# SimonsRoad/gf-pl-slam

Measured on AMD Instinct MI355X. Metric: stereo frames/sec (2k ORB + 500 LBD, 10 GN iters), higher is better.
Workload: dtype f64

## Files before the change

gf-pl-slam_amd/csrc/gfpl_knn.hpp:

```cpp
#pragma once
#include "gfpl_device.hpp"
#include "gfpl_layout.hpp"
#include <type_traits>

namespace gfpl {

typedef int mfma_v4i __attribute__((ext_vector_type(4)));
typedef int mfma_v8i __attribute__((ext_vector_type(8)));
typedef float mfma_v16f __attribute__((ext_vector_type(16)));

template <int CELL>
constexpr int knn_ksteps() { return (CELL == 2 ? 512 : 256) / 64; }

typedef mfma_v16f knn_acc_t;
constexpr float KNN_ACC_BIAS = 12582912.0f;
__device__ __forceinline__ uint32_t knn_acc_bits(float a) {
    return __float_as_uint(a);
}
__device__ __forceinline__ knn_acc_t knn_mma(mfma_v4i a, mfma_v4i b, knn_acc_t c) {
    const mfma_v8i a8 = __builtin_shufflevector(a, a, 0, 1, 2, 3, -1, -1, -1, -1);
    const mfma_v8i b8 = __builtin_shufflevector(b, b, 0, 1, 2, 3, -1, -1, -1, -1);
    return __builtin_amdgcn_mfma_scale_f32_32x32x64_f8f6f4(a8, b8, c, 4, 4, 0, 0x7F7F7F7F, 0, 0x7F7F7F7F);
}

__device__ __forceinline__ uint32_t fp4_cells2(uint32_t v) {
    return (2u << (4u * (v & 3u))) | (2u << (16u + 4u * ((v >> 2) & 3u)));
}
__device__ __forceinline__ uint32_t fp4_bits8(uint32_t b) {
    uint32_t x = b & 0xFFu;
    x = (x | (x << 12)) & 0x000F000Fu;
    x = (x | (x << 6)) & 0x03030303u;
    x = (x | (x << 3)) & 0x11111111u;
    return x << 1;
}

template <int CELL, bool SIGNED>
__device__ __forceinline__ mfma_v4i knn_frag(const uint32_t* d, int ks, int h) {
    mfma_v4i f;
    if (CELL == 2) {
        const uint32_t w = d[ks] >> (8u * (uint32_t)h);
#pragma unroll
        for (int i = 0; i < 4; ++i) {
            const uint32_t x = fp4_cells2((w >> (16 * (i >> 1) + 4 * (i & 1))) & 0xFu);
            f[i] = (int)(SIGNED ? x * 5u : x);
        }
    } else {
#pragma unroll
        for (int i = 0; i < 4; ++i) {
            const uint32_t x = fp4_bits8(d[2 * ks + (i >> 1)] >> (16u * (uint32_t)h + 8u * (i & 1)));
            f[i] = (int)(SIGNED ? (x << 2) | 0x22222222u : x);
        }
    }
    return f;
}

__device__ __forceinline__ int popc8(const uint32_t* d) {
    int s = 0;
#pragma unroll
    for (int i = 0; i < 8; ++i) s += __popc(d[i]);
    return s;
}

template <int CELL>
__device__ void knn_lut_fill(uint32_t* lut) {
    for (int b = threadIdx.x; b < 256; b += blockDim.x) {
        if (CELL == 2) {
            lut[2 * b] = fp4_cells2(b & 0xFu);
            lut[2 * b + 1] = fp4_cells2((uint32_t)b >> 4);
        } else {
            lut[b] = fp4_bits8(b);
        }
    }
}

template <int CELL>
__device__ __forceinline__ void knn_stage_views(uint32_t* T, int stride, const uint8_t* src, int nt) {
    constexpr uint32_t S0 = CELL == 2 ? 0x06040200u : 0x05040100u;
    constexpr uint32_t S1 = CELL == 2 ? 0x07050301u : 0x07060302u;
    const uint4* s4 = reinterpret_cast<const uint4*>(src);
    for (int k = threadIdx.x; k < nt * 2; k += blockDim.x) {
        const uint4 v = s4[k];
        const int t = k >> 1, j = (k & 1) * 2;
        T[(0 + j) * stride + t] = __builtin_amdgcn_perm(v.y, v.x, S0);
        T[(1 + j) * stride + t] = __builtin_amdgcn_perm(v.w, v.z, S0);
        T[(4 + j) * stride + t] = __builtin_amdgcn_perm(v.y, v.x, S1);
        T[(5 + j) * stride + t] = __builtin_amdgcn_perm(v.w, v.z, S1);
    }
}


__device__ __forceinline__ knn_acc_t knn_acc_init(int off) {
    knn_acc_t c;
#pragma unroll
    for (int r = 0; r < 16; ++r) c[r] = KNN_ACC_BIAS + (float)off;
    return c;
}

template <int CELL>
__device__ __forceinline__ uint32_t knn_query_offk(const uint32_t (&qd)[8]) {
    return (uint32_t)(CELL == 2 ? 128 : popc8(qd)) << 16;
}

template <int CELL>
__device__ __forceinline__ knn_acc_t knn_tile(const uint32_t* Th, int tstride, int rt, int c, int nt, const mfma_v4i* bq,
                                              knn_acc_t acc) {
    typedef uint32_t u32x2v __attribute__((ext_vector_type(2)));
    typedef __attribute__((address_space(3))) const u32x2v lds_cu2;
    typedef __attribute__((address_space(3))) const uint32_t lds_cu1;
    const int t = rt * 32 + c;
    uint32_t tv[4];
    if (rt * 32 + 32 <= nt) {
#pragma unroll
        for (int j = 0; j < 4; ++j) tv[j] = Th[j * tstride + t];
    } else if (t < nt) {
#pragma unroll
        for (int j = 0; j < 4; ++j) tv[j] = Th[j * tstride + t];
    } else {
#pragma unroll
        for (int j = 0; j < 4; ++j) tv[j] = 0;
    }
    auto ent = [&](int i, int sh) { return (uintptr_t)(((tv[i >> 2] >> (8 * (i & 3))) & 0xFFu) << sh); };
    mfma_v4i f[knn_ksteps<CELL>()];
#pragma unroll
    for (int ks = 0; ks < knn_ksteps<CELL>(); ++ks) {
        if (CELL == 2) {
            const u32x2v e0 = *reinterpret_cast<lds_cu2*>(ent(2 * ks, 3));
            const u32x2v e1 = *reinterpret_cast<lds_cu2*>(ent(2 * ks + 1, 3));
            f[ks][0] = (int)e0.x; f[ks][1] = (int)e0.y; f[ks][2] = (int)e1.x; f[ks][3] = (int)e1.y;
        } else {
#pragma unroll
            for (int i = 0; i < 4; ++i) f[ks][i] = (int)*reinterpret_cast<lds_cu1*>(ent(4 * ks + i, 2));
        }
    }
#pragma unroll
    for (int ks = 0; ks < knn_ksteps<CELL>(); ++ks) acc = knn_mma(f[ks], bq[ks], acc);
    return acc;
}

__device__ __forceinline__ uint32_t knn_acc_row(int r) { return (uint32_t)((r & 3) + 8 * (r >> 2)); }

__device__ __forceinline__ void knn_top2(uint32_t& k0, uint32_t& k1, uint32_t key) {
    asm("v_med3_u32 %0, %1, %2, %3" : "=v"(k1) : "v"(k0), "v"(k1), "v"(key));
    k0 = min(k0, key);
}

__device__ __forceinline__ void knn_merge_halves(uint32_t& k0, uint32_t& k1) {
    const uint32_t o0 = __shfl_xor(k0, 32, 64);
    const uint32_t o1 = __shfl_xor(k1, 32, 64);
    const uint32_t lo = min(k0, o0), hi0 = max(k0, o0);
    k1 = min(hi0, min(k1, o1));
    k0 = lo;
}

template <int CELL>
__device__ __forceinline__ void knn2_mfma(const uint32_t* T, int tstride, int nt, const uint8_t* Q, int nq, uint32_t* out_k0,
                                          uint32_t* out_k1, uint32_t* rl_key) {
    const int lane = threadIdx.x & 63;
    const int wave = threadIdx.x >> 6, nwave = blockDim.x >> 6;
    const int h = lane >> 5, c = lane & 31;
    const int nct = (nq + 31) >> 5, nrt = (nt + 31) >> 5;
    typedef uint32_t u32x2v __attribute__((ext_vector_type(2)));
    typedef __attribute__((address_space(3))) const u32x2v lds_cu2;
    typedef __attribute__((address_space(3))) const uint32_t lds_cu1;
    const uint32_t* Th = T + 4 * h * tstride;
    const int pr = lane & 15;
    const bool rb3 = (pr & 8) != 0, rb2 = (pr & 4) != 0, rb1 = (pr & 2) != 0, rb0 = (pr & 1) != 0;
    const uint32_t lro = (uint32_t)(4 * h + (pr & 3) + 8 * (pr >> 2));
    knn_acc_t acc0 = knn_acc_init(0);
#pragma unroll
    for (int r = 0; r < 16; ++r) asm volatile("" : "+v"(acc0[r]));
    for (int ct = wave; ct < nct; ct += nwave) {
        const int q = ct * 32 + c;
        uint32_t qd[8];
        if (q < nq) load_desc(Q + (size_t)q * 32, qd);
        else {
#pragma unroll
            for (int i = 0; i < 8; ++i) qd[i] = 0;
        }
        mfma_v4i bq[knn_ksteps<CELL>()];
#pragma unroll
        for (int ks = 0; ks < knn_ksteps<CELL>(); ++ks) {
            bq[ks] = knn_frag<CELL, true>(qd, ks, h);
        }
        const uint32_t offk = knn_query_offk<CELL>(qd);
        const uint32_t qo = offk + (q < nq ? (uint32_t)q : 0x7FFF0000u);
        uint32_t k0 = 0xFFFFFFFFu, k1 = 0xFFFFFFFFu;
        for (int rt = 0; rt < nrt; ++rt) {
            const int t = rt * 32 + c;
            uint32_t tv[4];
            if (rt * 32 + 32 <= nt) {
#pragma unroll
                for (int j = 0; j < 4; ++j) tv[j] = Th[j * tstride + t];
            } else if (t < nt) {
#pragma unroll
                for (int j = 0; j < 4; ++j) tv[j] = Th[j * tstride + t];
            } else {
#pragma unroll
                for (int j = 0; j < 4; ++j) tv[j] = 0;
            }
            knn_acc_t acc = acc0;
#pragma unroll
            for (int ks = 0; ks < knn_ksteps<CELL>(); ++ks) {
                auto ent = [&](int i, int sh) { return (uintptr_t)(((tv[i >> 2] >> (8 * (i & 3))) & 0xFFu) << sh); };
                mfma_v4i f;
                if (CELL == 2) {
                    const u32x2v e0 = *reinterpret_cast<lds_cu2*>(ent(2 * ks, 3));
                    const u32x2v e1 = *reinterpret_cast<lds_cu2*>(ent(2 * ks + 1, 3));
                    f[0] = (int)e0.x; f[1] = (int)e0.y; f[2] = (int)e1.x; f[3] = (int)e1.y;
                } else {
#pragma unroll
                    for (int i = 0; i < 4; ++i) f[i] = (int)*reinterpret_cast<lds_cu1*>(ent(4 * ks + i, 2));
                }
                acc = knn_mma(f, bq[ks], acc);
            }
            const uint32_t tb = (uint32_t)(rt * 32 + 4 * h);
            const uint32_t tko = offk + tb;
            auto epilogue = [&](auto chk_t) {
                constexpr bool chk = decltype(chk_t)::value;
                auto top2 = [&](int r, uint32_t sh) {
                    const uint32_t ro = knn_acc_row(r);
                    uint32_t key = sh + tko + ro;
                    if (chk && (int)(tb + ro) >= nt) key = 0xFFFFFFFFu;
                    knn_top2(k0, k1, key);
                };
                auto xchg = [](uint32_t a, uint32_t b, bool upper, auto ctrl_t) {
                    const uint32_t send = upper ? a : b, keep = upper ? b : a;
                    return min(keep, (uint32_t)__builtin_amdgcn_update_dpp(-1, (int)send, decltype(ctrl_t)::value, 0xF, 0xF, false));
                };
                uint32_t y[8];
#pragma unroll
                for (int j = 0; j < 8; ++j) {
                    const uint32_t s0 = knn_acc_bits(acc[j]) << 16, s1 = knn_acc_bits(acc[j + 8]) << 16;
                    top2(j, s0);
                    top2(j + 8, s1);
                    y[j] = xchg(s0 + qo, s1 + qo, rb3, std::integral_constant<int, 0x140>{});
                }
                uint32_t z[4];
#pragma unroll
                for (int j = 0; j < 4; ++j) z[j] = xchg(y[j], y[j + 4], rb2, std::integral_constant<int, 0x141>{});
                const uint32_t w0 = xchg(z[0], z[2], rb1, std::integral_constant<int, 0x1B>{});
                const uint32_t w1 = xchg(z[1], z[3], rb1, std::integral_constant<int, 0x1B>{});
                const uint32_t f = xchg(w0, w1, rb0, std::integral_constant<int, 0xB1>{});
                const uint32_t tr = (uint32_t)(rt * 32) + lro;
                if (!chk || (int)tr < nt) atomicMin(&rl_key[tr], f);
            };
            if (rt * 32 + 32 <= nt) epilogue(std::false_type{});
            else epilogue(std::true_type{});
        }
        knn_merge_halves(k0, k1);
        if (h == 0 && q < nq) {
            out_k0[q] = k0;
            out_k1[q] = k1;
        }
    }
}

}
```

gf-pl-slam_amd/csrc/k_cross.hip:

```cpp
#include "gfpl_kernels.hpp"
#include "gfpl_knn.hpp"

namespace gfpl {

struct CrossGrid {
    int gx, gy, ncell;
    double inv_cs;
};

__device__ __forceinline__ int grid_axis(double v, double inv_cs, int n) {
    double c = floor(v * inv_cs);
    c = c < 0.0 ? 0.0 : (c > (double)(n - 1) ? (double)(n - 1) : c);
    return (int)c;
}

__global__ void __launch_bounds__(64) k_predict_pose(KParams p) {
    const int b = blockIdx.x * 64 + threadIdx.x;
    if (b >= p.B) return;
    double T[16], A[16], Bm[16], Ti[16];
    for (int i = 0; i < 16; ++i) { A[i] = p.prev.pose.Tfw[16 * b + i]; Bm[i] = p.prev.pose.DT[16 * b + i]; }
    mat4_mul(A, Bm, T);
    mat4_inv(T, Ti);
    for (int i = 0; i < 16; ++i) {
        p.curr.pose.Tfw[16 * b + i] = T[i];
        p.scr.cross_tinv[16 * b + i] = Ti[i];
    }
}

#ifndef GFPL_CP_WAVES
#define GFPL_CP_WAVES 8
#endif
#ifndef GFPL_CP_XL
#define GFPL_CP_XL 1
#endif
template <bool XL>
__global__ void __launch_bounds__(1024, GFPL_CP_WAVES) k_cross_points(KParams p, CrossGrid G) {
    extern __shared__ __align__(16) unsigned char smem[];
    const int b = blockIdx.x;
    const int cap = p.kp_cap;
    const int NB = G.ncell + 1;
    const CrossPointsLds S(smem, cap, G.ncell, XL);
    double *const prevT = S.prevT, *const Tinv = S.Tinv;
    double2* const spxy = reinterpret_cast<double2*>(S.spxy);
    int *const cnt = S.cnt, *const start = S.start, *const sq = S.sq, *const lastT = S.lastT, *const misc = S.misc;
    float *const spx = S.spx, *const spy = S.spy;
    const int tid = threadIdx.x;
    const int Sp = p.prev.pt.n[b], Sc = p.curr.pt.n[b];
    if (tid < 16) {
        prevT[tid] = p.prev.pose.Tfw[16 * b + tid];
        Tinv[tid] = p.scr.cross_tinv[16 * b + tid];
    }
    for (int i = tid; i < NB; i += blockDim.x) cnt[i] = 0;
    __syncthreads();
    int total = 0;
    if (Sp > 0 && Sc > 0) {
        const DevPoints& P = p.prev.pt;
        const DevPoints& Cc = p.curr.pt;
        const size_t pb = (size_t)b * cap;
        double* proj = p.scr.proj + pb * 2;
        for (int q = tid; q < Sp; q += blockDim.x) {
            double v[4] = {P.P[3 * (pb + q)], P.P[3 * (pb + q) + 1], P.P[3 * (pb + q) + 2], 1.0};
            mat4_vec(prevT, v, v);
            mat4_vec(Tinv, v, v);
            double uv[2];
            projection(p.cam, v, uv);
            proj[2 * q] = uv[0];
            proj[2 * q + 1] = uv[1];
            int cell = G.ncell;
            if (uv[0] == uv[0] && uv[1] == uv[1])
                cell = grid_axis(uv[1], G.inv_cs, G.gy) * G.gx + grid_axis(uv[0], G.inv_cs, G.gx);
            lastT[q] = cell;
            atomicAdd(&cnt[cell], 1);
        }
        __syncthreads();
        int base = 0;
        for (int c0 = 0; c0 < NB; c0 += blockDim.x) {
            const int i = c0 + tid;
            const int v = i < NB ? cnt[i] : 0;
            int tot;
            const int r = base + block_exclusive_scan<1024>(v, misc, &tot);
            if (i < NB) start[i] = r;
            base += tot;
        }
        if (tid == 0) start[NB] = base;
        __syncthreads();
        for (int i = tid; i < NB; i += blockDim.x) cnt[i] = 0;
        __syncthreads();
        for (int q = tid; q < Sp; q += blockDim.x) {
            const int cell = lastT[q];
            const int pos = start[cell] + atomicAdd(&cnt[cell], 1);
            sq[pos] = q;
            const double ux = proj[2 * q], uy = proj[2 * q + 1];
            spx[pos] = (float)ux;
            spy[pos] = (float)uy;
            if (XL) spxy[pos] = make_double2(ux, uy);
            lastT[q] = -1;
        }
        __syncthreads();
        const double gate = p.cfg.proj_gate_px;
        const float fpre = (float)(gate + 1.5);
        const float radius = (float)p.cfg.point_match_radius;
        const int cap_m = p.cfg.max_point_match_num;
        const uint8_t* PD = P.desc + pb * 32;
        int off = 0;
        for (int c0 = 0; c0 < Sc; c0 += blockDim.x) {
            const int t = c0 + tid;
            int bestq = -1;
            if (t < Sc) {
                const double plx = Cc.pl[2 * (pb + t)], ply = Cc.pl[2 * (pb + t) + 1];
                uint32_t dt[8];
                load_desc(Cc.desc + (pb + t) * 32, dt);
                int bestd = 0x7FFFFFFF;
                auto consider_at = [&](int q, double ux, double uy) {
                    const double dx = ux - plx, dy = uy - ply;
                    if (sqrt(dx * dx + dy * dy) > gate) return;
                    uint32_t dq[8];
                    load_desc(PD + (size_t)q * 32, dq);
                    const int d = hamming8<1>(dq, dt);
                    if ((float)d <= radius && (d < bestd || (d == bestd && q < bestq))) { bestd = d; bestq = q; }
                };
                auto consider = [&](int q) { consider_at(q, proj[2 * q], proj[2 * q + 1]); };
                auto consider_k = [&](int k) {
                    if (XL) {
                        const double2 u = spxy[k];
                        consider_at(sq[k], u.x, u.y);
                    } else {
                        consider(sq[k]);
                    }
                };
                const bool normal = fabs(plx) < 1e6 && fabs(ply) < 1e6;
                if (normal) {
                    const float fx = (float)plx, fy = (float)ply;
                    const int cx = grid_axis(plx, G.inv_cs, G.gx), cy = grid_axis(ply, G.inv_cs, G.gy);
                    const int x0 = max(cx - 1, 0), x1 = min(cx + 1, G.gx - 1);
                    for (int yy = max(cy - 1, 0); yy <= min(cy + 1, G.gy - 1); ++yy) {
                        const int k1 = start[yy * G.gx + x1 + 1];
                        for (int k = start[yy * G.gx + x0]; k < k1; ++k) {
                            if (fabsf(spx[k] - fx) > fpre || fabsf(spy[k] - fy) > fpre) continue;
                            consider_k(k);
                        }
                    }
                    for (int k = start[G.ncell]; k < start[NB]; ++k) consider_k(k);
                } else {
                    for (int q = 0; q < Sp; ++q) consider(q);
                }
            }
            const int has = bestq >= 0 ? 1 : 0;
            int tot;
            const int rank = off + block_exclusive_scan<1024>(has, misc, &tot);
            if (has && rank < cap_m) {
                p.tr.matched_pt[(size_t)b * p.mpt_cap + rank] = bestq;
                Cc.idx[pb + t] = P.idx[pb + bestq];
                atomicMax(&lastT[bestq], t);
            }
            off += tot;
            if (off >= cap_m) break;
        }
        total = off < cap_m ? off : cap_m;
        __syncthreads();
        for (int q = tid; q < Sp; q += blockDim.x) {
            const int t = lastT[q];
            if (t >= 0) {
                P.pl_obs[2 * (pb + q)] = Cc.pl[2 * (pb + t)];
                P.pl_obs[2 * (pb + q) + 1] = Cc.pl[2 * (pb + t) + 1];
                P.inlier[pb + q] = 1;
            }
        }
    }
    if (tid == 0) {
        p.tr.n_matched_pt[b] = total;
        p.tr.n_inliers_pt[b] = total;
        p.tr.n_inliers[b] = total + p.tr.n_matched_ls[b];
    }
}

#ifndef GFPL_CL_WAVES
#define GFPL_CL_WAVES 1
#endif
template <int BLOCK>
__global__ void __launch_bounds__(BLOCK, GFPL_CL_WAVES) k_cross_lines(KParams p) {
    extern __shared__ __align__(16) unsigned char smem[];
    const int b = blockIdx.x;
    const int cap = p.kl_cap;
    uint32_t* lut = (uint32_t*)smem;
    uint32_t* tb = lut + knn_lut_dwords(1);
    int* i12 = (int*)(tb + cap * 8);
    int* d012 = i12 + cap;
    int* d112 = d012 + cap;
    int* i21 = d112 + cap;
    int* h12 = i21 + cap;
    int* h0 = h12 + 260;
    int* misc = h0 + 260;
    const int tid = threadIdx.x;
    const int Sl = p.prev.ls.n[b], Sc = p.curr.ls.n[b];
    int total = 0;
    if (Sl >= 2 && Sc >= 2) {
        DevLines& P = p.prev.ls;
        DevLines& Cc = p.curr.ls;
        const size_t pb = (size_t)b * cap;
        const uint8_t* DP = P.desc + pb * 32;
        const uint8_t* DC = Cc.desc + pb * 32;
        knn_stage_views<1>(tb, cap, DC, Sc);
        for (int i = tid; i < 520; i += blockDim.x) h12[i] = 0;
        for (int j = tid; j < Sc; j += blockDim.x) i21[j] = -1;
        knn_lut_fill<1>(lut);
        __syncthreads();
        knn2_mfma<1>(tb, cap, Sc, DP, Sl, (uint32_t*)i12, (uint32_t*)d112, (uint32_t*)i21);
        __syncthreads();
        for (int i = tid; i < Sl; i += blockDim.x) {
            const uint32_t k0 = (uint32_t)i12[i], k1 = (uint32_t)d112[i];
            const int d0 = (int)(k0 >> 16), d1 = (int)(k1 >> 16);
            i12[i] = (int)(k0 & 0xFFFFu); d012[i] = d0; d112[i] = d1;
            atomicAdd(&h12[d1 - d0], 1);
            atomicAdd(&h0[d0], 1);
        }
        for (int j = tid; j < Sc; j += blockDim.x) i21[j] = (int)((uint32_t)i21[j] & 0xFFFFu);
        __syncthreads();
        if (tid < 128) {
            if (tid < 64) {
                const int v = wave_hist_rank(h12, Sl / 2, 257);
                if (tid == 0) reinterpret_cast<double*>(misc + 16)[0] = (1.4826 * (double)(float)v) * p.cfg.desc_th_l;
            } else {
                const int k = min(p.cfg.max_line_match_num, Sl) - 1;
                const int v = wave_hist_rank(h0, k, 257);
                if (tid == 64) reinterpret_cast<double*>(misc + 16)[1] = (double)(float)v;
            }
        }
        __syncthreads();
        const double nn12 = reinterpret_cast<double*>(misc + 16)[0];
        const double budget = reinterpret_cast<double*>(misc + 16)[1];
        const int cap_m = p.cfg.max_line_match_num;
        int off = 0;
        for (int c0 = 0; c0 < Sl; c0 += BLOCK) {
            const int i = c0 + tid;
            int acc = 0, t = 0;
            if (i < Sl) {
                t = i12[i];
                const int rl = i21[t];
                const bool over = (double)(float)d012[i] > 1.2 * budget;
                const double dist_12 = (double)((float)d112[i] - (float)d012[i]);
                acc = (!over && i == rl && dist_12 > nn12) ? 1 : 0;
            }
            int tot;
            const int rank = off + block_exclusive_scan<BLOCK>(acc, misc, &tot);
            if (acc && rank < cap_m) {
                const size_t qi = pb + i, qt = pb + t;
                P.sdisp_obs[qi] = Cc.sdisp[qt];
                P.edisp_obs[qi] = Cc.edisp[qt];
                P.spl_obs[2 * qi] = Cc.spl[2 * qt]; P.spl_obs[2 * qi + 1] = Cc.spl[2 * qt + 1];
                P.epl_obs[2 * qi] = Cc.epl[2 * qt]; P.epl_obs[2 * qi + 1] = Cc.epl[2 * qt + 1];
                for (int k = 0; k < 3; ++k) P.le_obs[3 * qi + k] = Cc.le[3 * qt + k];
                P.inlier[qi] = 1;
                p.tr.matched_ls[(size_t)b * p.mls_cap + rank] = i;
                Cc.idx[qt] = P.idx[qi];
            }
            off += tot;
            if (off >= cap_m) break;
        }
        total = off < cap_m ? off : cap_m;
    }
    if (tid == 0) {
        p.tr.n_matched_ls[b] = total;
        p.tr.n_inliers_ls[b] = total;
        p.tr.n_inliers[b] = p.tr.n_inliers_pt[b] + total;
    }
}

CrossGrid cross_grid(const KParams& p) {
    const double pre = p.cfg.proj_gate_px + 0.5;
    int cs = 16;
    CrossGrid G;
    for (;;) {
        G.gx = (p.cam.width + cs - 1) / cs;
        G.gy = (p.cam.height + cs - 1) / cs;
        if ((double)cs >= pre && G.gx * G.gy <= 2048) break;
        cs *= 2;
    }
    G.ncell = G.gx * G.gy;
    G.inv_cs = 1.0 / cs;
    return G;
}

hipError_t launch_cross_points(const KParams& p, hipStream_t s) {
    const CrossGrid G = cross_grid(p);
    hipLaunchKernelGGL(k_predict_pose, dim3((p.B + 63) / 64), dim3(64), 0, s, p);
    const size_t lxl = CrossPointsLds(nullptr, p.kp_cap, G.ncell, true).bytes;
    static std::atomic<unsigned long long> attr[2];
    if (GFPL_CP_XL && p.kp_cap <= 2048 && lxl <= 80 * 1024) {
        const hipError_t e = ensure_dyn_lds(reinterpret_cast<const void*>(k_cross_points<true>), DYN_LDS_CEILING, &attr[1]);
        if (e != hipSuccess) return e;
        hipLaunchKernelGGL(k_cross_points<true>, dim3(p.B), dim3(1024), lxl, s, p, G);
    } else {
        const hipError_t e = ensure_dyn_lds(reinterpret_cast<const void*>(k_cross_points<false>), DYN_LDS_CEILING, &attr[0]);
        if (e != hipSuccess) return e;
        hipLaunchKernelGGL(k_cross_points<false>, dim3(p.B), dim3(1024),
                           CrossPointsLds(nullptr, p.kp_cap, G.ncell, false).bytes, s, p, G);
    }
    return hipGetLastError();
}

hipError_t launch_cross_lines(const KParams& p, hipStream_t s) {
    const size_t lds = CrossLinesLds(nullptr, p.kl_cap).bytes;
    if (p.kl_cap > 1024 || p.B <= sp_wide_max_b()) {
        static std::atomic<unsigned long long> attr{0};
        const hipError_t e = ensure_dyn_lds(reinterpret_cast<const void*>(k_cross_lines<1024>), DYN_LDS_CEILING, &attr);
        if (e != hipSuccess) return e;
        hipLaunchKernelGGL(k_cross_lines<1024>, dim3(p.B), dim3(1024), lds, s, p);
    } else
        hipLaunchKernelGGL(k_cross_lines<512>, dim3(p.B), dim3(512), lds, s, p);
    return hipGetLastError();
}

}
```

gf-pl-slam_amd/csrc/k_stereo.hip:

```cpp
#include <type_traits>

#include "gfpl_kernels.hpp"
#include "gfpl_knn.hpp"

namespace gfpl {

template <typename K>
__device__ void bitonic_sort(K* a, int n) {
    for (int k = 2; k <= n; k <<= 1)
        for (int j = k >> 1; j > 0; j >>= 1) {
            for (int i = threadIdx.x; i < n; i += blockDim.x) {
                int ixj = i ^ j;
                if (ixj > i) {
                    bool up = ((i & k) == 0);
                    K x = a[i], y = a[ixj];
                    if ((x > y) == up) { a[i] = y; a[ixj] = x; }
                }
            }
            __syncthreads();
        }
}

template <typename K>
__device__ void bitonic_sort2(K* a, K* c, int n) {
// ... 514 lines not shown
            J.lvl = p.cam.lvl_offset[J.o];
            J.scaleduR0 = (float)J.uR;
#ifdef GFPL_SP_PROBE_SAMEWIN
            J.o = 0; J.vL = 20; J.uL = 60; J.uR = 40;
            J.cols = p.cam.lvl_cols[0]; J.lvl = p.cam.lvl_offset[0];
#endif
            sad_rows(J, q, acc);
        }
#pragma unroll
        for (int s = 0; s < 11; ++s) {
            uint32_t v = acc[s];
            v += (uint32_t)__builtin_amdgcn_update_dpp(0, (int)v, 0xB1, 0xF, 0xF, false);
            v += (uint32_t)__builtin_amdgcn_update_dpp(0, (int)v, 0x4E, 0xF, 0xF, false);
            acc[s] = v;
        }
        if (job != 0xFFFFFFFFu && q == 0) {
            const int iL = (int)(job & 0xFFFFu);
            float disparity = -1, bestuR;
            sad_finish(p, J, xL, acc, disparity, bestuR);
            uint32_t key = 0xFFFFFFFFu;
            if (disparity >= minD && disparity < maxD) {
                if (disparity <= 0) { disparity = 0.01f; bestuR = (float)((double)xL - 0.01); }
                depth[iL] = mbf / disparity;
                key = ((pr & 0x7Fu) << 16) | (uint32_t)iL;
            }
            pairs[iL] = key;
        }
    }
    __syncthreads();
    SP_CLK(4);
    SP_PRIO(0);
    uint32_t* keys = pairs;
    if (SEG) {
        constexpr int NW = BLOCK / 64;
        int* cnt = reinterpret_cast<int*>(stg);
        int* wcnt = cnt + 128;
        for (int x = tid; x < 128 * (NW + 1); x += BLOCK) cnt[x] = 0;
        __syncthreads();
        for (int i = tid; i < N; i += BLOCK) {
            const uint32_t k = pairs[i];
            if (k != 0xFFFFFFFFu) atomicAdd(&cnt[k >> 16], 1);
        }
        __syncthreads();
        if (tid < 64) {
            const int c0 = cnt[2 * tid], c1 = cnt[2 * tid + 1];
            int x = c0 + c1;
#pragma unroll
            for (int o = 1; o < 64; o <<= 1) {
                const int y = __shfl_up(x, o, 64);
                if (tid >= o) x += y;
            }
            const int ex = x - (c0 + c1);
            cnt[2 * tid] = ex;
            cnt[2 * tid + 1] = ex + c0;
            if (tid == 63) misc[1] = x;
        }
        __syncthreads();
        const int wave = tid >> 6, lane = tid & 63;
        const unsigned long long lt = (1ull << lane) - 1ull;
        keys = order;
        for (int r0 = 0; r0 < N; r0 += BLOCK) {
            const int i = r0 + tid;
            const uint32_t k = i < N ? pairs[i] : 0xFFFFFFFFu;
            const bool v = k != 0xFFFFFFFFu;
            const int d = (int)(k >> 16) & 127;
            unsigned long long peers = __ballot(v);
#pragma unroll
            for (int bit = 0; bit < 7; ++bit) {
                const bool on = (d >> bit) & 1;
                const unsigned long long m = __ballot(on);
                peers &= on ? m : ~m;
            }
            const int rnk = __popcll(peers & lt);
            if (v && rnk == 0) wcnt[wave * 128 + d] = __popcll(peers);
            __syncthreads();
            if (v) {
                int pos = cnt[d] + rnk;
                for (int w = 0; w < wave; ++w) pos += wcnt[w * 128 + d];
                keys[pos] = k;
            }
            __syncthreads();
            if (tid < 128) {
                int sum = 0;
#pragma unroll
                for (int w = 0; w < NW; ++w) { sum += wcnt[w * 128 + tid]; wcnt[w * 128 + tid] = 0; }
                cnt[tid] += sum;
            }
            __syncthreads();
        }
    } else {
        bitonic_sort(pairs, KP2);
        for (int i = tid; i < KP2; i += blockDim.x) {
            bool v = pairs[i] != 0xFFFFFFFFu;
            bool vn = (i + 1 < KP2) ? (pairs[i + 1] != 0xFFFFFFFFu) : false;
            if (v && !vn) misc[1] = i + 1;
        }
        __syncthreads();
    }
    const int nv = misc[1];
    float thDist = 0.0f;
    if (nv > 0) {
        const float median = (float)(keys[nv / 2] >> 16);
        thDist = 1.5f * 1.4f * median;
    }
    DevPoints& C = p.curr.pt;
    const size_t base = (size_t)b * cap;
    int off = 0;
    for (int c0 = 0; c0 < nv; c0 += BLOCK) {
        const int i = c0 + tid;
        int flag = 0;
        float disparity = 0.0f;
        int iL = 0;
        if (i < nv) {
            const uint32_t k = keys[i];
            const int dist = (int)(k >> 16);
            iL = (int)(k & 0xFFFFu);
            if ((float)dist < thDist) {
                disparity = mbf / depth[iL];
                flag = (disparity < 0) ? 0 : 1;
            }
        }
        int tot;
        const int pos = off + block_exclusive_scan<BLOCK>(flag, misc + 4, &tot);
        if (flag) {
            const gfpl_keypoint kp = KL[iL];
            const size_t q = base + pos;
            const double plx = kp.x, ply = kp.y, disp = (double)disparity;
            double P[3];
            backProjection(p.cam, plx, ply, disp, P);
            C.pl[2 * q] = plx; C.pl[2 * q + 1] = ply;
            C.disp[q] = disp;
            C.P[3 * q] = P[0]; C.P[3 * q + 1] = P[1]; C.P[3 * q + 2] = P[2];
            const int lv = clamp_level(kp.octave, p.cam.n_levels);
            C.sigma2[q] = p.cam.sigma2_pt[lv];
            C.idx[q] = pos;
            C.level[q] = kp.octave;
            C.inlier[q] = 1;
            const uint4* s = reinterpret_cast<const uint4*>(DL + (size_t)iL * 32);
            uint4* d = reinterpret_cast<uint4*>(C.desc + q * 32);
            d[0] = s[0]; d[1] = s[1];
        }
        off += tot;
    }
    if (tid == 0) {
        C.n[b] = off;
        p.curr.pose.time_stamp[b] = p.in.time_stamp[b];
        p.scr.n_subpix[b] = misc[2];
    }
    SP_CLK(5);
}

#ifndef GFPL_SL_PRIO
#define GFPL_SL_PRIO 1
#endif
#if GFPL_SL_PRIO
#define SL_PRIO(k) __builtin_amdgcn_s_setprio(k)
#else
#define SL_PRIO(k) do { } while (0)
#endif
struct LineOut {
    double spl[2], epl[2], sdisp, edisp, sP[3], eP[3], le[3], angle;
    int level;
};

__device__ __forceinline__ int eig_gate_bound(const double* C, double th) {
    double M = 0.0, G = -__builtin_inf(), D = -__builtin_inf();
    bool fin = true;
#pragma unroll
    for (int i = 0; i < 9; ++i) { fin = fin && (C[i] - C[i] == 0.0); M = fmax(M, fabs(C[i])); }
    if (!fin) return -1;
#pragma unroll
    for (int i = 0; i < 3; ++i) {
        const double d = C[4 * i];
        const double r = (d + fabs(C[3 * i + (i + 1) % 3])) + fabs(C[3 * i + (i + 2) % 3]);
        G = fmax(G, r);
        D = fmax(D, d);
    }
    if (D >= th) return 0;
    if (G + 4e-9 * M < th) return 1;
    return -1;
}

__device__ bool triangulate(const KParams& p, const gfpl_keyline& a, const gfpl_keyline& c, bool initial,
                            LineOut* L) {
    const DevCam& cam = p.cam;
    double sp_l[3] = {a.sx, a.sy, 1.0}, ep_l[3] = {a.ex, a.ey, 1.0};
    double le_l[3] = {sp_l[1] * ep_l[2] - sp_l[2] * ep_l[1], sp_l[2] * ep_l[0] - sp_l[0] * ep_l[2],
                      sp_l[0] * ep_l[1] - sp_l[1] * ep_l[0]};
    double nrm = sqrt(le_l[0] * le_l[0] + le_l[1] * le_l[1]);
    le_l[0] = le_l[0] / nrm; le_l[1] = le_l[1] / nrm; le_l[2] = le_l[2] / nrm;
    double sp_r[3] = {c.sx, c.sy, 1.0}, ep_r[3] = {c.ex, c.ey, 1.0};
    double le_r[3] = {sp_r[1] * ep_r[2] - sp_r[2] * ep_r[1], sp_r[2] * ep_r[0] - sp_r[0] * ep_r[2],
                      sp_r[0] * ep_r[1] - sp_r[1] * ep_r[0]};
    double overlap = overlapStereo(sp_l[1], ep_l[1], sp_r[1], ep_r[1]);
    double spx = (-(le_r[2] + le_r[1] * (double)a.sy)) / le_r[0];
    double epx = (-(le_r[2] + le_r[1] * (double)a.ey)) / le_r[0];
    double disp_s = (double)a.sx - spx;
    double disp_e = (double)a.ex - epx;
    double horiz = initial ? (double)fabsf((float)le_r[0]) : (double)fabsf((float)le_l[0]);
    if (!(disp_s >= p.cfg.min_disp && disp_e >= p.cfg.min_disp && horiz > p.cfg.line_horiz_th &&
          overlap > p.cfg.stereo_overlap_th))
        return false;
    if (!initial) {
        double cS[9], cE[9];
        endpointCov(cam, sp_l[0], sp_l[1], disp_s, cS);
        endpointCov(cam, ep_l[0], ep_l[1], disp_e, cE);
        const double th = p.cfg.line_cov_th;
        const int gS = eig_gate_bound(cS, th), gE = eig_gate_bound(cE, th);
        if (gS == 0 || gE == 0) return false;
        if (!(gS == 1 && gE == 1)) {
            double wS[3], wE[3];
            eig_sym<3>(cS, wS);
            eig_sym<3>(cE, wE);
            double max_eig = std_max(wS[2], wE[2]);
            if (!(max_eig < th)) return false;
        }
    }
    L->spl[0] = sp_l[0]; L->spl[1] = sp_l[1];
    L->epl[0] = ep_l[0]; L->epl[1] = ep_l[1];
    L->sdisp = disp_s; L->edisp = disp_e;
    backProjection(cam, sp_l[0], sp_l[1], disp_s, L->sP);
    backProjection(cam, ep_l[0], ep_l[1], disp_e, L->eP);
    L->le[0] = le_l[0]; L->le[1] = le_l[1]; L->le[2] = le_l[2];
    L->angle = (double)a.angle;
    L->level = a.octave;
    return true;
}

__device__ void line_uncertainty(const KParams& p, const double* spl, const double* epl, double sdisp,
                                 double edisp, const double* le, double* covS, double* covE) {
    double sdisp_std, edisp_std;
    if (fabs(le[0]) > 0.15) {
        sdisp_std = p.cfg.ratio_disp_std * sdisp;
        edisp_std = p.cfg.ratio_disp_std * edisp;
    } else {
        sdisp_std = p.cfg.ratio_disp_std_hor * sdisp;
        edisp_std = p.cfg.ratio_disp_std_hor * edisp;
    }
    covMat2D_3D(p.cam, spl[0], spl[1], 1.0, sdisp, sdisp_std, covS);
    covMat2D_3D(p.cam, epl[0], epl[1], 1.0, edisp, edisp_std, covE);
}

__device__ void write_line(const KParams& p, DevLines& C, size_t q, const LineOut& L, int idx, const uint8_t* desc) {
    C.spl[2 * q] = L.spl[0]; C.spl[2 * q + 1] = L.spl[1];
    C.epl[2 * q] = L.epl[0]; C.epl[2 * q + 1] = L.epl[1];
    C.sdisp[q] = L.sdisp; C.edisp[q] = L.edisp;
    for (int k = 0; k < 3; ++k) { C.sP[3 * q + k] = L.sP[k]; C.eP[3 * q + k] = L.eP[k]; C.le[3 * q + k] = L.le[k]; }
    C.angle[q] = L.angle;
    C.level[q] = L.level;
    C.sigma2[q] = p.cam.sigma2_ln[clamp_level(L.level, GFPL_MAX_LEVELS)];
    C.idx[q] = idx;
    C.inlier[q] = 1;
    C.cut[2 * q] = 0.0; C.cut[2 * q + 1] = 0.0;
    const uint4* s = reinterpret_cast<const uint4*>(desc);
    uint4* d = reinterpret_cast<uint4*>(C.desc + q * 32);
    d[0] = s[0]; d[1] = s[1];
}

#ifdef GFPL_SL_CLOCK
#define SL_CLK(k) do { if (threadIdx.x == 0 && !INITIAL) p.scr.dbg[8 * (size_t)blockIdx.x + (k)] = (int64_t)wall_clock64(); } while (0)
#else
#define SL_CLK(k) do { } while (0)
#endif
template <int CELL, bool INITIAL, int BLOCK>
__global__ void __launch_bounds__(BLOCK, GFPL_SL_WAVES) k_stereo_lines(KParams p) {
    extern __shared__ __align__(16) unsigned char smem[];
    const int b = blockIdx.x;
    const int cap = p.kl_cap;
    uint32_t* lut = (uint32_t*)smem;
    uint32_t* tb = lut + knn_lut_dwords(CELL);
    int* lr_i = (int*)(tb + cap * 8);
    int* lr_d0 = lr_i + cap;
    int* lr_d1 = lr_d0 + cap;
    int* rl_i = lr_d1 + cap;
    int* hist = rl_i + cap;
    int* misc = hist + 260;
    const int tid = threadIdx.x;
    const int NL = min(p.in.n_kl_l[b], cap), NR = min(p.in.n_kl_r[b], cap);
    DevLines& C = p.curr.ls;
    if (NL < 2 || NR < 2) {
        if (tid == 0) C.n[b] = 0;
        return;
    }
    const uint8_t* DLg = p.in.ldesc_l + (size_t)b * cap * 32;
    const uint8_t* DRg = p.in.ldesc_r + (size_t)b * cap * 32;
    SL_CLK(0);
    SL_PRIO(3);
    knn_stage_views<CELL>(tb, cap, DRg, NR);
    for (int i = tid; i < 260; i += blockDim.x) hist[i] = 0;
    for (int j = tid; j < NR; j += blockDim.x) rl_i[j] = -1;
    knn_lut_fill<CELL>(lut);
    __syncthreads();
    SL_CLK(1);
    knn2_mfma<CELL>(tb, cap, NR, DLg, NL, (uint32_t*)lr_i, (uint32_t*)lr_d1, (uint32_t*)rl_i);
    __syncthreads();
    SL_CLK(2);
    SL_PRIO(1);
    for (int i = tid; i < NL; i += blockDim.x) {
        const uint32_t k0 = (uint32_t)lr_i[i], k1 = (uint32_t)lr_d1[i];
        const int d0 = (int)(k0 >> 16), d1 = (int)(k1 >> 16);
        lr_i[i] = (int)(k0 & 0xFFFFu); lr_d0[i] = d0; lr_d1[i] = d1;
        atomicAdd(&hist[d1 - d0], 1);
    }
    for (int j = tid; j < NR; j += blockDim.x) rl_i[j] = (int)((uint32_t)rl_i[j] & 0xFFFFu);
    __syncthreads();
    if (tid < 64) {
        const int v = wave_hist_rank(hist, NL / 2, 257);
        if (tid == 0) {
            double th = (1.4826 * (double)(float)v) * p.cfg.desc_th_l;
            reinterpret_cast<double*>(misc + 8)[0] = th;
        }
    }
    __syncthreads();
    const double nn12_dist_th = reinterpret_cast<double*>(misc + 8)[0];
    SL_CLK(3);
    const int n_matches = min(NL, NR);
    const gfpl_keyline* KL = p.in.kl_l + (size_t)b * cap;
    const gfpl_keyline* KR = p.in.kl_r + (size_t)b * cap;
    const size_t base = (size_t)b * cap;
    int off = 0;
    for (int c0 = 0; c0 < n_matches; c0 += BLOCK) {
        const int i = c0 + tid;
        int flag = 0;
        LineOut L;
        if (i < n_matches) {
            const int lr_tdx = lr_i[i];
            const int rl_tdx = rl_i[lr_tdx];
            const double dist_12 = (double)((float)lr_d1[i] - (float)lr_d0[i]);
            if (i == rl_tdx && dist_12 > nn12_dist_th)
                flag = triangulate(p, KL[i], KR[lr_tdx], INITIAL, &L) ? 1 : 0;
        }
        int tot;
        const int pos = off + block_exclusive_scan<BLOCK>(flag, misc + 16, &tot);
        if (flag) write_line(p, C, base + pos, L, INITIAL ? pos : -1, DLg + (size_t)i * 32);
        off += tot;
    }
    if (tid == 0) C.n[b] = off;
    SL_CLK(4);
}

__global__ void __launch_bounds__(512) k_init_points(KParams p) {
    __shared__ int misc[32];
    const int b = blockIdx.x;
    const int cap = p.kp_cap;
    const int tid = threadIdx.x;
    DevPoints& C = p.curr.pt;
    const int N = min(p.in.n_kp_l[b], cap), Nr = min(p.in.n_kp_r[b], cap);
    if (N < 2 || Nr < 2) {
        if (tid == 0) { C.n[b] = 0; p.curr.pose.time_stamp[b] = p.in.time_stamp[b]; }
        return;
    }
    const int32_t* lr = p.scr.knn + (size_t)b * 2 * cap * 3;
    const int32_t* rl = lr + (size_t)cap * 3;
    const gfpl_keypoint* KL = p.in.kp_l + (size_t)b * cap;
    const gfpl_keypoint* KR = p.in.kp_r + (size_t)b * cap;
    const uint8_t* DL = p.in.pdesc_l + (size_t)b * cap * 32;
    const size_t base = (size_t)b * cap;
    int off = 0;
    for (int c0 = 0; c0 < N; c0 += 512) {
        const int i = c0 + tid;
        int flag = 0;
        double disp_ = 0.0;
        if (i < N) {
            const int t = lr[3 * i];
            const int rl_tdx = rl[3 * t];
            const double dist_12 = (double)((float)lr[3 * i + 1] / (float)lr[3 * i + 2]);
            if (i == rl_tdx && dist_12 <= p.cfg.max_ratio_12_p) {
                const gfpl_keypoint kl = KL[i], kr = KR[t];
                if ((double)fabsf(kl.y - kr.y) <= p.cfg.max_dist_epip) {
                    disp_ = (double)(kl.x - kr.x);
                    if (disp_ >= p.cfg.min_disp) flag = 1;
                }
            }
        }
        int tot;
        const int pos = off + block_exclusive_scan<512>(flag, misc, &tot);
        if (flag) {
            const gfpl_keypoint kl = KL[i];
            const size_t q = base + pos;
            double P[3];
            const double plx = kl.x, ply = kl.y;
            backProjection(p.cam, plx, ply, disp_, P);
            C.pl[2 * q] = plx; C.pl[2 * q + 1] = ply;
            C.disp[q] = disp_;
            C.P[3 * q] = P[0]; C.P[3 * q + 1] = P[1]; C.P[3 * q + 2] = P[2];
            C.sigma2[q] = p.cam.sigma2_pt[clamp_level(kl.octave, p.cam.n_levels)];
            C.idx[q] = pos;
            C.level[q] = kl.octave;
            C.inlier[q] = 1;
            const uint4* s = reinterpret_cast<const uint4*>(DL + (size_t)i * 32);
            uint4* d = reinterpret_cast<uint4*>(C.desc + q * 32);
            d[0] = s[0]; d[1] = s[1];
        }
        off += tot;
    }
    if (tid == 0) {
        C.n[b] = off;
        p.curr.pose.time_stamp[b] = p.in.time_stamp[b];
    }
}

__global__ void k_init_pose(KParams p) {
    const int b = blockIdx.x * blockDim.x + threadIdx.x;
    if (b >= p.B) return;
    DevPose& P = p.curr.pose;
    for (int i = 0; i < 16; ++i) { P.Tfw[16 * b + i] = (i % 5 == 0) ? 1.0 : 0.0; P.DT[16 * b + i] = (i % 5 == 0) ? 1.0 : 0.0; }
    for (int i = 0; i < 36; ++i) { P.Tfw_cov[36 * b + i] = (i % 7 == 0) ? 1.0 : 0.0; P.DT_cov[36 * b + i] = 0.0; }
    for (int i = 0; i < 6; ++i) P.DT_cov_eig[6 * b + i] = 0.0;
    P.err_norm[b] = 0.0;
    p.tr.num_frame_loss[b] = 0;
    p.tr.n_matched_pt[b] = 0;
    p.tr.n_matched_ls[b] = 0;
    p.tr.n_inliers[b] = 0; p.tr.n_inliers_pt[b] = 0; p.tr.n_inliers_ls[b] = 0;
    for (int i = 0; i < 16; ++i) p.tr.kf_T[16 * b + i] = (i % 5 == 0) ? 1.0 : 0.0;
    for (int i = 0; i < 36; ++i) p.tr.kf_cov[36 * b + i] = 0.0;
    p.tr.kf_prev_iskf[b] = 1;
    p.tr.kf_nsince[b] = 0;
    p.tr.kf_entropy0[b] = 0.0;
    p.tr.kf_ratio[b] = 0.0;
    p.tr.kf_flag[b] = 0;
}

__global__ void __launch_bounds__(256) k_line_uncertainty(KParams p) {
    __shared__ double cs[256 * 9], ce[256 * 9];
    const int b = blockIdx.y;
    const int i0 = blockIdx.x * blockDim.x;
    const int i = i0 + threadIdx.x;
    DevLines& L = p.prev.ls;
    const int n = L.n[b];
    if (i0 >= n) return;
    if (i < n) {
        const size_t q = (size_t)b * p.kl_cap + i;
        double spl[2] = {L.spl[2 * q], L.spl[2 * q + 1]}, epl[2] = {L.epl[2 * q], L.epl[2 * q + 1]};
        double le[3] = {L.le[3 * q], L.le[3 * q + 1], L.le[3 * q + 2]};
        double cS[9], cE[9];
        line_uncertainty(p, spl, epl, L.sdisp[q], L.edisp[q], le, cS, cE);
#pragma unroll
        for (int k = 0; k < 9; ++k) { cs[9 * threadIdx.x + k] = cS[k]; ce[9 * threadIdx.x + k] = cE[k]; }
    }
    __syncthreads();
    const int m = 9 * min(256, n - i0);
    double* dS = L.covS + 9 * ((size_t)b * p.kl_cap + i0);
    double* dE = L.covE + 9 * ((size_t)b * p.kl_cap + i0);
    for (int k = threadIdx.x; k < m; k += 256) { dS[k] = cs[k]; dE[k] = ce[k]; }
}

__global__ void k_step_bytes(KParams p) {
    const int b = blockIdx.x * blockDim.x + threadIdx.x;
    if (b >= p.B) return;
    const int64_t No = (int64_t)p.in.n_kp_l[b] + p.in.n_kp_r[b];
    const int64_t Nk = (int64_t)p.in.n_kl_l[b] + p.in.n_kl_r[b];
    const int64_t Mo = p.scr.n_subpix[b];
    const int64_t Sp = p.prev.pt.n[b], Sl = p.prev.ls.n[b];
    const int64_t Sp2 = p.curr.pt.n[b], Sl2 = p.curr.ls.n[b];
    const int64_t Mp = p.tr.n_matched_pt[b], Ml = p.tr.n_matched_ls[b];
    int64_t st[6];
    st[0] = 44 * No + (121 + 231) * Mo + 97 * Sp2;
    st[1] = 56 * Nk + 193 * Sl2;
    st[2] = 216 * Sl + 60 * Sp + 48 * Sp2 + 25 * Mp + 256;
    st[3] = 36 * Sl + 32 * Sl2 + 153 * Ml;
    st[4] = 608 * Ml + 44 * Mp;
    st[5] = 54 * Mp + 86 * Ml + 1504;
    int64_t tot = 0;
    int64_t* rec = p.scr.bytes + (size_t)STEP_REC * b;
    for (int i = 0; i < 6; ++i) { rec[i] = st[i]; tot += st[i]; }
    rec[6] = tot;
    rec[7] = (p.cfg.use_line_conf_cut && Ml > 0) ? 396 * Ml + 272 : 0;
    rec[8] = No; rec[9] = Nk; rec[10] = Mo; rec[11] = Sp2; rec[12] = Sl2; rec[13] = Mp; rec[14] = Ml;
    rec[15] = p.tr.n_inliers[b];
    if (!(p.cfg.use_line_conf_cut && Ml > 0)) rec[16] = rec[17] = 0;
    rec[18] = rec[15];
    if (!(p.cfg.use_line_conf_cut && Ml > 0)) rec[19] = 0;
    if (!(p.cfg.use_line_conf_cut && p.cfg.cut_with_max_vol && (p.cfg.cut_proof == 1 || p.cfg.cut_proof == 3)))
        rec[20] = rec[21] = rec[22] = rec[23] = 0;
    p.tr.kf_nsince[b] = p.tr.kf_nsince[b] + 1;
}

static inline int next_pow2(int v) { int p = 1; while (p < v) p <<= 1; return p; }

#ifndef SP_WIDE_MAX_B
#define SP_WIDE_MAX_B 256
#endif
int sp_wide_max_b() {
    const char* e = getenv("GFPL_SP_WIDE_MAX_B");
    return e ? atoi(e) : SP_WIDE_MAX_B;
}

hipError_t launch_stereo_points(const KParams& p, hipStream_t s) {
    const int KP2 = next_pow2(p.kp_cap);
    auto lds_of = [&](bool seg, int waves) {
        return (size_t)StereoPointsLds(nullptr, KP2, p.cam.height, p.cam.n_levels, seg, waves).bytes;
    };
    const size_t lds_seg = lds_of(true, 8), lds_seg_w = lds_of(true, 16);
    if (p.B <= sp_wide_max_b() && p.kp_cap <= 2048 && lds_seg_w <= 64 * 1024) {
        hipLaunchKernelGGL((k_stereo_points<1024, true>), dim3(p.B), dim3(1024), lds_seg_w, s, p, KP2);
        return hipGetLastError();
    }
    if (p.kp_cap > 2048) {
        static std::atomic<unsigned long long> attr{0};
        const hipError_t e = ensure_dyn_lds(reinterpret_cast<const void*>(k_stereo_points<1024, false>), DYN_LDS_CEILING, &attr);
        if (e != hipSuccess) return e;
        hipLaunchKernelGGL((k_stereo_points<1024, false>), dim3(p.B), dim3(1024), lds_of(false, 16), s, p, KP2);
    }
    else if (lds_seg <= 54 * 1024 && p.kp_cap <= 2048)
        hipLaunchKernelGGL((k_stereo_points<512, true>), dim3(p.B), dim3(512), lds_seg, s, p, KP2);
    else
        hipLaunchKernelGGL((k_stereo_points<512, false>), dim3(p.B), dim3(512), lds_of(false, 8), s, p, KP2);
    return hipGetLastError();
}

template <int CELL, bool INITIAL, int BLOCK>
static hipError_t launch_stereo_lines_as(const KParams& p, hipStream_t s) {
    if (BLOCK == 1024) {
        static std::atomic<unsigned long long> attr{0};
        const hipError_t e = ensure_dyn_lds(reinterpret_cast<const void*>(k_stereo_lines<CELL, INITIAL, BLOCK>),
                                            DYN_LDS_CEILING, &attr);
        if (e != hipSuccess) return e;
    }
    hipLaunchKernelGGL((k_stereo_lines<CELL, INITIAL, BLOCK>), dim3(p.B), dim3(BLOCK),
                       StereoLinesLds(nullptr, p.kl_cap, CELL).bytes, s, p);
    return hipGetLastError();
}

hipError_t launch_stereo_lines(const KParams& p, hipStream_t s) {
    if (p.kl_cap > 1024 || p.B <= sp_wide_max_b()) return launch_stereo_lines_as<2, false, 1024>(p, s);
    return launch_stereo_lines_as<2, false, 512>(p, s);
}

hipError_t launch_line_uncertainty(const KParams& p, hipStream_t s) {
    hipLaunchKernelGGL(k_line_uncertainty, dim3((p.kl_cap + 255) / 256, p.B), dim3(256), 0, s, p);
    return hipGetLastError();
}

hipError_t launch_init(const KParams& p, hipStream_t s) {
    const int cap = p.kp_cap;
    int32_t* lr = p.scr.knn;
    hipError_t e = launch_knn2_batched(p.in.pdesc_l, p.in.n_kp_l, p.in.pdesc_r, p.in.n_kp_r, cap, p.B, 1, lr, s);
    if (e != hipSuccess) return e;
    e = launch_knn2_batched(p.in.pdesc_r, p.in.n_kp_r, p.in.pdesc_l, p.in.n_kp_l, cap, p.B, 1, lr + (size_t)cap * 3, s);
    if (e != hipSuccess) return e;
    hipLaunchKernelGGL(k_init_points, dim3(p.B), dim3(512), 0, s, p);
    e = p.kl_cap > 1024 ? launch_stereo_lines_as<1, true, 1024>(p, s) : launch_stereo_lines_as<1, true, 512>(p, s);
    if (e != hipSuccess) return e;
    hipLaunchKernelGGL(k_init_pose, dim3((p.B + 63) / 64), dim3(64), 0, s, p);
    return hipGetLastError();
}

hipError_t launch_step_bytes(const KParams& p, hipStream_t s) {
    hipLaunchKernelGGL(k_step_bytes, dim3((p.B + 63) / 64), dim3(64), 0, s, p);
    return hipGetLastError();
}

}
```

Measured before the change: 791,700.

## Fold match-key packing into MFMA accumulator via block scale and float bias

```diff
diff --git a/gf-pl-slam_amd/csrc/gfpl_knn.hpp b/gf-pl-slam_amd/csrc/gfpl_knn.hpp
--- a/gf-pl-slam_amd/csrc/gfpl_knn.hpp
+++ b/gf-pl-slam_amd/csrc/gfpl_knn.hpp
@@ -17,10 +17,12 @@
 __device__ __forceinline__ uint32_t knn_acc_bits(float a) {
     return __float_as_uint(a);
 }
+template <int S>
 __device__ __forceinline__ knn_acc_t knn_mma(mfma_v4i a, mfma_v4i b, knn_acc_t c) {
+    static_assert(S >= 0 && S < 32, "block scale 2^S");
     const mfma_v8i a8 = __builtin_shufflevector(a, a, 0, 1, 2, 3, -1, -1, -1, -1);
     const mfma_v8i b8 = __builtin_shufflevector(b, b, 0, 1, 2, 3, -1, -1, -1, -1);
-    return __builtin_amdgcn_mfma_scale_f32_32x32x64_f8f6f4(a8, b8, c, 4, 4, 0, 0x7F7F7F7F, 0, 0x7F7F7F7F);
+    return __builtin_amdgcn_mfma_scale_f32_32x32x64_f8f6f4(a8, b8, c, 4, 4, 0, 0x7F7F7F7F + S * 0x01010101, 0, 0x7F7F7F7F);
 }
 
 __device__ __forceinline__ uint32_t fp4_cells2(uint32_t v) {
@@ -133,7 +135,7 @@
         }
     }
 #pragma unroll
-    for (int ks = 0; ks < knn_ksteps<CELL>(); ++ks) acc = knn_mma(f[ks], bq[ks], acc);
+    for (int ks = 0; ks < knn_ksteps<CELL>(); ++ks) acc = knn_mma<0>(f[ks], bq[ks], acc);
     return acc;
 }
 
@@ -151,6 +153,52 @@
     k1 = min(hi0, min(k1, o1));
     k0 = lo;
 }
+
+constexpr int KNN_KEY_S = 13;
+constexpr int KNN_KEY_R0 = 2016;
+constexpr int KNN_KEY_CAP = 2048;
+constexpr int KNN_KEY_COUNT = 256;
+constexpr uint32_t KNN_KEY_BASE = 0x4B400000u;
+constexpr uint32_t KNN_KEY_PAD = 0x40000000u;
+constexpr uint32_t KNN_IDX_MASK = (1u << KNN_KEY_S) - 1u;
+static_assert(KNN_KEY_R0 >= 32 * ((KNN_KEY_CAP + 31) / 32 - 1), "a tile-relative row field would borrow from the count");
+static_assert(KNN_KEY_R0 + 31 + (KNN_KEY_CAP - 1) < (1 << KNN_KEY_S), "row field + query index would carry into the count");
+static_assert((KNN_KEY_COUNT << KNN_KEY_S) <= (1 << 22), "1.5 * 2^23 - 256 * 2^S must stay >= 2^23");
+static_assert((KNN_KEY_COUNT << KNN_KEY_S) + (1 << KNN_KEY_S) <= (1 << 22), "1.5 * 2^23 + 256 * 2^S + row field must stay < 2^24");
+static_assert(KNN_KEY_BASE + (1u << 22) + KNN_KEY_PAD < 0xFFFFFFFFu - 32u * 64u, "pad keys and aged sentinels stay apart");
+
+template <int CELL>
+__device__ __forceinline__ uint32_t knn_query_off(const uint32_t (&qd)[8]) {
+    return (uint32_t)(CELL == 2 ? 128 : popc8(qd));
+}
+
+__device__ __forceinline__ uint32_t knn_key_decode(uint32_t k, uint32_t off, int nrt) {
+    const uint32_t u = k - KNN_KEY_BASE + (off << KNN_KEY_S);
+    const uint32_t t = (u & KNN_IDX_MASK) + (uint32_t)(32 * (nrt - 1) - KNN_KEY_R0);
+    return k >= 0x80000000u ? 0xFFFFFFFFu : ((u >> KNN_KEY_S) << 16) | t;
+}
+
+#define GFPL_KNN_XCHG4(CTRL, LO, HI)                                              \
+    "v_min_u32_dpp %0, %0, %0 " CTRL " row_mask:0xf bank_mask:" LO "\n\t"         \
+    "v_min_u32_dpp %0, %4, %4 " CTRL " row_mask:0xf bank_mask:" HI "\n\t"         \
+    "v_min_u32_dpp %1, %1, %1 " CTRL " row_mask:0xf bank_mask:" LO "\n\t"         \
+    "v_min_u32_dpp %1, %5, %5 " CTRL " row_mask:0xf bank_mask:" HI "\n\t"         \
+    "v_min_u32_dpp %2, %2, %2 " CTRL " row_mask:0xf bank_mask:" LO "\n\t"         \
+    "v_min_u32_dpp %2, %6, %6 " CTRL " row_mask:0xf bank_mask:" HI "\n\t"         \
+    "v_min_u32_dpp %3, %3, %3 " CTRL " row_mask:0xf bank_mask:" LO "\n\t"         \
+    "v_min_u32_dpp %3, %7, %7 " CTRL " row_mask:0xf bank_mask:" HI
+__device__ __forceinline__ void knn_xchg4_mirror(uint32_t* a, uint32_t* b, uint32_t qo, uint32_t k0, uint32_t k1) {
+    asm("v_add_u32 %0, %0, %8\n\tv_add_u32 %4, %4, %8\n\tv_add_u32 %1, %1, %8\n\tv_add_u32 %5, %5, %8\n\t"
+        "v_add_u32 %2, %2, %8\n\tv_add_u32 %6, %6, %8\n\tv_add_u32 %3, %3, %8\n\tv_add_u32 %7, %7, %8\n\t"
+        GFPL_KNN_XCHG4("row_mirror", "0x3", "0xc")
+        : "+v"(a[0]), "+v"(a[1]), "+v"(a[2]), "+v"(a[3]), "+v"(b[0]), "+v"(b[1]), "+v"(b[2]), "+v"(b[3])
+        : "v"(qo), "v"(k0), "v"(k1));
+}
+__device__ __forceinline__ void knn_xchg4_half_mirror(uint32_t* a, const uint32_t* b) {
+    asm("s_nop 1\n\t" GFPL_KNN_XCHG4("row_half_mirror", "0x5", "0xa")
+        : "+v"(a[0]), "+v"(a[1]), "+v"(a[2]), "+v"(a[3]) : "v"(b[0]), "v"(b[1]), "v"(b[2]), "v"(b[3]));
+}
+#undef GFPL_KNN_XCHG4
 
 template <int CELL>
 __device__ __forceinline__ void knn2_mfma(const uint32_t* T, int tstride, int nt, const uint8_t* Q, int nq, uint32_t* out_k0,
@@ -164,9 +212,12 @@
     typedef __attribute__((address_space(3))) const uint32_t lds_cu1;
     const uint32_t* Th = T + 4 * h * tstride;
     const int pr = lane & 15;
-    const bool rb3 = (pr & 8) != 0, rb2 = (pr & 4) != 0, rb1 = (pr & 2) != 0, rb0 = (pr & 1) != 0;
+    const bool rb1 = (pr & 2) != 0, rb0 = (pr & 1) != 0;
     const uint32_t lro = (uint32_t)(4 * h + (pr & 3) + 8 * (pr >> 2));
-    knn_acc_t acc0 = knn_acc_init(0);
+    const uint32_t rsub = (uint32_t)KNN_KEY_R0 + lro;
+    knn_acc_t acc0;
+#pragma unroll
+    for (int r = 0; r < 16; ++r) acc0[r] = KNN_ACC_BIAS + (float)(KNN_KEY_R0 + (int)knn_acc_row(r) + 4 * h);
 #pragma unroll
     for (int r = 0; r < 16; ++r) asm volatile("" : "+v"(acc0[r]));
     for (int ct = wave; ct < nct; ct += nwave) {
@@ -182,8 +233,8 @@
         for (int ks = 0; ks < knn_ksteps<CELL>(); ++ks) {
             bq[ks] = knn_frag<CELL, true>(qd, ks, h);
         }
-        const uint32_t offk = knn_query_offk<CELL>(qd);
-        const uint32_t qo = offk + (q < nq ? (uint32_t)q : 0x7FFF0000u);
+        const uint32_t off = knn_query_off<CELL>(qd);
+        const uint32_t qo = (off << KNN_KEY_S) + (q < nq ? (uint32_t)q : KNN_KEY_PAD);
         uint32_t k0 = 0xFFFFFFFFu, k1 = 0xFFFFFFFFu;
         for (int rt = 0; rt < nrt; ++rt) {
             const int t = rt * 32 + c;
@@ -211,48 +262,48 @@
 #pragma unroll
                     for (int i = 0; i < 4; ++i) f[i] = (int)*reinterpret_cast<lds_cu1*>(ent(4 * ks + i, 2));
                 }
-                acc = knn_mma(f, bq[ks], acc);
+                acc = knn_mma<KNN_KEY_S>(f, bq[ks], acc);
             }
             const uint32_t tb = (uint32_t)(rt * 32 + 4 * h);
-            const uint32_t tko = offk + tb;
+            k0 -= 32u;
+            k1 -= 32u;
             auto epilogue = [&](auto chk_t) {
                 constexpr bool chk = decltype(chk_t)::value;
-                auto top2 = [&](int r, uint32_t sh) {
-                    const uint32_t ro = knn_acc_row(r);
-                    uint32_t key = sh + tko + ro;
-                    if (chk && (int)(tb + ro) >= nt) key = 0xFFFFFFFFu;
+                auto top2 = [&](int r) {
+                    uint32_t key = knn_acc_bits(acc[r]);
+                    if (chk && (int)(tb + knn_acc_row(r)) >= nt) key = 0xFFFFFFFFu;
                     knn_top2(k0, k1, key);
                 };
                 auto xchg = [](uint32_t a, uint32_t b, bool upper, auto ctrl_t) {
                     const uint32_t send = upper ? a : b, keep = upper ? b : a;
                     return min(keep, (uint32_t)__builtin_amdgcn_update_dpp(-1, (int)send, decltype(ctrl_t)::value, 0xF, 0xF, false));
                 };
-                uint32_t y[8];
+                uint32_t y[8], yb[8];
 #pragma unroll
                 for (int j = 0; j < 8; ++j) {
-                    const uint32_t s0 = knn_acc_bits(acc[j]) << 16, s1 = knn_acc_bits(acc[j + 8]) << 16;
-                    top2(j, s0);
-                    top2(j + 8, s1);
-                    y[j] = xchg(s0 + qo, s1 + qo, rb3, std::integral_constant<int, 0x140>{});
+                    top2(j);
+                    top2(j + 8);
+                    y[j] = knn_acc_bits(acc[j]);
+                    yb[j] = knn_acc_bits(acc[j + 8]);
                 }
-                uint32_t z[4];
-#pragma unroll
-                for (int j = 0; j < 4; ++j) z[j] = xchg(y[j], y[j + 4], rb2, std::integral_constant<int, 0x141>{});
-                const uint32_t w0 = xchg(z[0], z[2], rb1, std::integral_constant<int, 0x1B>{});
-                const uint32_t w1 = xchg(z[1], z[3], rb1, std::integral_constant<int, 0x1B>{});
+                knn_xchg4_mirror(y, yb, qo, k0, k1);
+                knn_xchg4_mirror(y + 4, yb + 4, qo, k0, k1);
+                knn_xchg4_half_mirror(y, y + 4);
+                const uint32_t w0 = xchg(y[0], y[2], rb1, std::integral_constant<int, 0x1B>{});
+                const uint32_t w1 = xchg(y[1], y[3], rb1, std::integral_constant<int, 0x1B>{});
                 const uint32_t f = xchg(w0, w1, rb0, std::integral_constant<int, 0xB1>{});
                 const uint32_t tr = (uint32_t)(rt * 32) + lro;
-                if (!chk || (int)tr < nt) atomicMin(&rl_key[tr], f);
+                if (!chk || (int)tr < nt) atomicMin(&rl_key[tr], f - rsub);
             };
             if (rt * 32 + 32 <= nt) epilogue(std::false_type{});
             else epilogue(std::true_type{});
         }
         knn_merge_halves(k0, k1);
         if (h == 0 && q < nq) {
-            out_k0[q] = k0;
-            out_k1[q] = k1;
-        }
-    }
-}
-
-}
+            out_k0[q] = knn_key_decode(k0, off, nrt);
+            out_k1[q] = knn_key_decode(k1, off, nrt);
+        }
+    }
+}
+
+}
diff --git a/gf-pl-slam_amd/csrc/k_cross.hip b/gf-pl-slam_amd/csrc/k_cross.hip
--- a/gf-pl-slam_amd/csrc/k_cross.hip
+++ b/gf-pl-slam_amd/csrc/k_cross.hip
@@ -214,7 +214,7 @@
             atomicAdd(&h12[d1 - d0], 1);
             atomicAdd(&h0[d0], 1);
         }
-        for (int j = tid; j < Sc; j += blockDim.x) i21[j] = (int)((uint32_t)i21[j] & 0xFFFFu);
+        for (int j = tid; j < Sc; j += blockDim.x) i21[j] = (int)((uint32_t)i21[j] & KNN_IDX_MASK);
         __syncthreads();
         if (tid < 128) {
             if (tid < 64) {
diff --git a/gf-pl-slam_amd/csrc/k_stereo.hip b/gf-pl-slam_amd/csrc/k_stereo.hip
--- a/gf-pl-slam_amd/csrc/k_stereo.hip
+++ b/gf-pl-slam_amd/csrc/k_stereo.hip
@@ -840,7 +840,7 @@
         lr_i[i] = (int)(k0 & 0xFFFFu); lr_d0[i] = d0; lr_d1[i] = d1;
         atomicAdd(&hist[d1 - d0], 1);
     }
-    for (int j = tid; j < NR; j += blockDim.x) rl_i[j] = (int)((uint32_t)rl_i[j] & 0xFFFFu);
+    for (int j = tid; j < NR; j += blockDim.x) rl_i[j] = (int)((uint32_t)rl_i[j] & KNN_IDX_MASK);
     __syncthreads();
     if (tid < 64) {
         const int v = wave_hist_rank(hist, NL / 2, 257);
```

Measured after the change: 806,700 (median of 6 runs). 1.02x the previous value.
